# MarineRoboticsGroup/mac

Hardware: AMD Instinct MI355X
Metric: frank_wolfe_iters_per_sec (higher is better)
Workload: dtype f64; 1 GPU; configs[3]: ER N=100000 ~2M candidates, chain fixed, K=10%; N=100000, m_candidates=2001737, K=200173, fixed_edges=99999, fw_iters=209, parallelism=single GPU

## Files before the change

mac_amd/csrc/kernels.h:

```cpp
#pragma once
#include "common.h"

namespace machip {

template <typename T>
struct CsrViewT {
    int n;
    const int* rowptr;
    const int* col;
    const T* val;
};
using CsrView = CsrViewT<double>;

struct PatternView {
    int n;
    const int* prow;
    const int* pcol;
    const int* pk;
    const double* pw;
};

struct LanState {
    int jA;
    int jB;
// ... 17 lines not shown
};

constexpr int kAsmGrid = 4096;
__global__ __launch_bounds__(kBlock) void k_x_bits(const double* __restrict__ x, long m, double tol, unsigned long long* __restrict__ bits) {
    for (long i = (long)blockIdx.x * kBlock + threadIdx.x; i < m; i += (long)gridDim.x * kBlock) {
        const unsigned long long bal = __ballot(x[i] > tol);
        if ((threadIdx.x & 63) == 0) bits[i >> 6] = bal;
    }
}
__device__ __forceinline__ bool x_bit(const unsigned int* __restrict__ bits32, int k) { return (bits32[k >> 5] >> (k & 31)) & 1u; }

template <int G>
__global__ __launch_bounds__(kBlock) void k_asm_count(PatternView P, const unsigned int* __restrict__ xbits,
                                                      int rows_per_block,
                                                      int* __restrict__ cnt, int* __restrict__ blk_sum,
                                                      int* __restrict__ hsum = nullptr) {
    __shared__ int sm[4];
    constexpr int GPB = kBlock / G;
    const int lane = threadIdx.x % G, g = threadIdx.x / G;
    const int r0 = blockIdx.x * rows_per_block;
    const int r1 = min(P.n, r0 + rows_per_block);
    int local = 0, supp = 0, mx = 0;
    for (int r = r0 + g; r < r1; r += GPB) {
        const int b = P.prow[r], e = P.prow[r + 1];
        int c = 0, sc = 0;
        for (int p = b + lane; p < e; p += G) {
            const int k = P.pk[p];
            const bool cand = k >= 0;
            const bool act = cand ? x_bit(xbits, k) : true;
            c += act;
            sc += (cand && act);
        }
// ... 296 lines not shown
    double mx;
    __device__ __forceinline__ void begin(double*) { mx = 0.0; }
    __device__ __forceinline__ double gather(const double* __restrict__ x, int c) const { return x[c]; }
    __device__ __forceinline__ void row(int r, double acc) {
        const double d = dg[r];
        double v = d > 0.0 ? uin[r] + (1.0 - acc) / d : 0.0;
        v = v > 0.0 && v < 1e300 ? v : 0.0;
        uout[r] = v;
        mx = fmax(mx, v);
    }
    __device__ __forceinline__ void end(double* sm) {
        const double m = block_max(mx, sm);
        if (threadIdx.x == 0) pmax[blockIdx.x] = m;
    }
};
__global__ __launch_bounds__(kBlock) void k_land_weight(const double* __restrict__ u, const double* __restrict__ pmax, int npart,
                                                        double* __restrict__ z, int n, double p, double floor_w) {
    __shared__ double sm[4];
    double m = 0.0;
    for (int i = threadIdx.x; i < npart; i += kBlock) m = fmax(m, pmax[i]);
    m = block_max(m, sm);
    if (!(m > 0.0)) return;
    const double inv = 1.0 / m;
    for (int r = blockIdx.x * kBlock + threadIdx.x; r < n; r += gridDim.x * kBlock) {
        const double q = u[r] * inv;
        z[r] *= fmax(q > 0.0 ? exp(p * log(q)) : 0.0, floor_w);
    }
}

__global__ __launch_bounds__(kBlock) void k_lan_update(LanView L) {
    __shared__ double sm[4];
    const int j = L.st->jB;
    const double alpha = reduce_partials(L.part_a, L.P_a, sm);
    const double beta = L.beta[j];
    const double* vj = L.V + (size_t)j * (size_t)L.n;
    const double* vp = j > 0 ? vj - L.n : nullptr;
    double s1 = 0.0, s2 = 0.0, s3 = 0.0;
    for (int r = blockIdx.x * kBlock + threadIdx.x; r < L.n; r += gridDim.x * kBlock) {
        double t = L.w[r] - alpha * vj[r];
        if (vp) t -= beta * vp[r];
        L.u[r] = t;
// ... 658 lines not shown
            else { if (run) atomicAdd(&lh[cur], run); cur = bin; run = 1; }
        }
    }
    if (HIST) {
        if (run) atomicAdd(&lh[cur], run);
        __syncthreads();
        unsigned int* hr = hist0 + (size_t)(blockIdx.x % kSelRep) * kBins;
        for (int i = threadIdx.x; i < kBins; i += kBlock)
            if (lh[i]) atomicAdd(&hr[i], lh[i]);
    }
    if (all.n) peer_drain();
}

template <int BLOCK, class LoadBin>
__device__ __forceinline__ void sel_close_pass(LoadBin load_bin, int pass, unsigned long long prefix, SelState* st,
                                               unsigned int* s_w ) {
    const int tid = threadIdx.x, wv = tid >> 6, ln = tid & 63;
    const int sh = sel_shift(pass), nb = sel_bits(pass);
    const long long kk = pass ? st->kk : st->k;
    const int nbins = 1 << nb;
    constexpr int per = kBins / BLOCK;
    unsigned int c[per];
    unsigned int tsum = 0;
#pragma unroll
    for (int q = 0; q < per; ++q) {
        const int bin = nbins - 1 - (tid * per + q);
        c[q] = bin >= 0 ? load_bin(bin) : 0u;
        tsum += c[q];
    }
    unsigned int x = tsum;
    for (int o = 1; o < 64; o <<= 1) { const unsigned int y = __shfl_up(x, o, kWave); if (ln >= o) x += y; }
    __syncthreads();
    if (ln == 63) s_w[wv] = x;
    __syncthreads();
    for (int q = 0; q < wv; ++q) x += s_w[q];
    const long long pre = (long long)x;
    if (pre >= kk && pre - (long long)tsum < kk) {
        long long rem = kk - (pre - (long long)tsum);
        int q = 0;
        for (; q < per; ++q) {
            if ((long long)c[q] >= rem) break;
            rem -= c[q];
        }
        const int bin = nbins - 1 - (tid * per + q);
        st->kk = rem;
        st->prefix = (prefix << nb) | (unsigned long long)bin;
        if (pass == 5) {
            st->T = (prefix << nb) | (unsigned long long)bin;
            st->cnt_eq = (long long)c[q];
        } else if ((long long)c[q] == rem) {
            st->T = ((prefix << nb) | (unsigned long long)bin) << sh;
            st->cnt_eq = rem;
            st->ticket[7] = 1u;
        }
    }
}

__global__ __launch_bounds__(1024) void k_sel_close0(unsigned int* __restrict__ hist, SelState* st) {
    __shared__ unsigned int s_w[1024 / 64];
    if (st->k <= 0) return;
    const unsigned int* rep = hist + 6 * kBins;
    sel_close_pass<1024>([rep](int bin) {
        unsigned int v[kSelRep];
#pragma unroll
        for (int r = 0; r < kSelRep; ++r) v[r] = rep[(size_t)r * kBins + bin];
        unsigned int a = 0;
#pragma unroll
        for (int r = 0; r < kSelRep; ++r) a += v[r];
        return a; }, 0, 0ull, st, s_w);
}

template <int U, int BLOCK>
__global__ __launch_bounds__(BLOCK) void k_sel_pass(const double* __restrict__ g, long m, int pass,
                                                    unsigned int* __restrict__ hist ,
                                                    SelState* st) {
    __shared__ unsigned int lh[kBins];
    __shared__ unsigned int s_last;
    __shared__ unsigned int s_w[BLOCK / 64];
    const int tid = threadIdx.x;
    if (pass && st->ticket[7]) return;
    for (int i = tid; i < kBins; i += BLOCK) lh[i] = 0;
    __syncthreads();
    const int sh = sel_shift(pass), nb = sel_bits(pass);
    const unsigned long long prefix = pass ? st->prefix : 0ull;
    const unsigned int mask = (1u << nb) - 1u;
    unsigned int cur = 0xffffffffu, run = 0;
    for (long i0 = (long)blockIdx.x * (BLOCK * U) + tid; i0 < m; i0 += (long)gridDim.x * (BLOCK * U)) {
        double gv[U];
#pragma unroll
        for (int q = 0; q < U; ++q) { const long i = i0 + (long)q * BLOCK; gv[q] = g[i < m ? i : m - 1]; }
#pragma unroll
        for (int q = 0; q < U; ++q) {
            if (i0 + (long)q * BLOCK >= m) continue;
            const unsigned long long key = f64_key(gv[q]);
            const bool match = pass == 0 || (key >> (sh + nb)) == prefix;
            if (match) {
                const unsigned int bin = (unsigned int)(key >> sh) & mask;
                if (bin == cur) ++run;
                else {
                    if (run) atomicAdd(&lh[cur], run);
                    cur = bin; run = 1;
                }
            }
        }
    }
    if (run) atomicAdd(&lh[cur], run);
    __syncthreads();
    unsigned int* gh = hist + pass * kBins;
    unsigned int seen = 0;
    for (int i = tid; i < kBins; i += BLOCK)
        if (lh[i]) seen |= __hip_atomic_fetch_add(&gh[i], lh[i], __ATOMIC_RELAXED, __HIP_MEMORY_SCOPE_AGENT);
    asm volatile("" ::"v"(seen));
    __syncthreads();
    if (tid == 0)
        s_last = (__hip_atomic_fetch_add(&st->ticket[pass], 1u, __ATOMIC_ACQ_REL, __HIP_MEMORY_SCOPE_AGENT) == gridDim.x - 1);
    __syncthreads();
    if (!s_last) return;
    sel_close_pass<BLOCK>([gh](int bin) { return __hip_atomic_load(&gh[bin], __ATOMIC_RELAXED, __HIP_MEMORY_SCOPE_AGENT); }, pass, prefix, st, s_w);
}

__global__ __launch_bounds__(1024) void k_sel_ties(const double* __restrict__ g, long m, SelState* st, int prefer_high) {
    __shared__ int s_cnt[16];
    __shared__ long long s_found;
    const long long need = st->kk;
    const long long eq = st->cnt_eq;
    if (st->k <= 0) { if (threadIdx.x == 0) st->tie_limit = prefer_high ? 0x7fffffffffffffffll : -1; return; }
    if (need >= eq) { if (threadIdx.x == 0) st->tie_limit = prefer_high ? -1 : 0x7fffffffffffffffll; return; }
    const unsigned long long T = st->T;
    const int tid = threadIdx.x, wv = tid >> 6, ln = tid & 63;
    if (tid == 0) s_found = -1;
    long long run = 0;
    for (long base = 0; base < m; base += 1024) {
        const long ii = base + tid;
        const long i = prefer_high ? m - 1 - ii : ii;
        const bool is = ii < m && f64_key(g[i]) == T;
        const unsigned long long bal = __ballot(is);
        __syncthreads();
        if (ln == 0) s_cnt[wv] = __popcll(bal);
        __syncthreads();
        int before = 0, tot = 0;
        for (int q = 0; q < 16; ++q) { if (q < wv) before += s_cnt[q]; tot += s_cnt[q]; }
        if (run + tot >= need) {
            const int rank = before + __popcll(bal & ((1ull << ln) - 1ull));
            if (is && run + rank + 1 == need) s_found = i;
            __syncthreads();
            if (tid == 0) st->tie_limit = s_found;
            return;
        }
        run += tot;
    }
    if (tid == 0) st->tie_limit = prefer_high ? -1 : 0x7fffffffffffffffll;
}

constexpr long kSelSmallMax = 32768;
__global__ __launch_bounds__(1024) void k_sel_small(const double* __restrict__ g, long m, long long k, SelState* st, int prefer_high) {
    __shared__ unsigned int lh[kBins];
    __shared__ unsigned int s_w[16];
    __shared__ unsigned long long s_prefix, s_T;
    __shared__ long long s_kk, s_eq, s_found;
    __shared__ int s_done, s_cnt[16];
    const int tid = threadIdx.x, wv = tid >> 6, ln = tid & 63;
    if (tid == 0) { s_prefix = 0; s_T = 0; s_kk = k; s_eq = 0; s_done = 0; s_found = -1; }
    __syncthreads();
    for (int pass = 0; pass < 6 && k > 0; ++pass) {
        if (s_done) break;
        for (int i = tid; i < kBins; i += 1024) lh[i] = 0;
// ... 55 lines not shown
        int before = 0, tot = 0;
        for (int q = 0; q < 16; ++q) { if (q < wv) before += s_cnt[q]; tot += s_cnt[q]; }
        if (runs + tot >= need) {
            const int rank = before + __popcll(bal & ((1ull << ln) - 1ull));
            if (is && runs + rank + 1 == need) s_found = i;
            __syncthreads();
            if (tid == 0) st->tie_limit = s_found;
            return;
        }
        runs += tot;
    }
    if (tid == 0) st->tie_limit = prefer_high ? -1 : 0x7fffffffffffffffll;
}

__global__ __launch_bounds__(kBlock) void k_fw_final(const double* __restrict__ g, const double* __restrict__ x,
                                                     long m, const SelState* __restrict__ st, double gamma,
                                                     double* __restrict__ x_next, double* __restrict__ s_out,
                                                     double* __restrict__ part ,
                                                     double tol = 0.0, unsigned long long* __restrict__ xbits_next = nullptr) {
#pragma clang fp contract(off)
    __shared__ double sm[4];
    const unsigned long long T = st->T;
    const long long lim = st->tie_limit;
    const bool none = st->k <= 0;
    double d = 0.0, q = 0.0;
    for (long i = (long)blockIdx.x * kBlock + threadIdx.x; i < m; i += (long)gridDim.x * kBlock) {
        const double gi = g[i];
        const unsigned long long key = f64_key(gi);
        const double s = (!none && (key > T || (key == T && (long long)i <= lim))) ? 1.0 : 0.0;
        if (s_out) s_out[i] = s;
        if (x) {
            const double xi = x[i];
            const double diff = s - xi;
            d += gi * diff;
            q += gi * gi;
            if (x_next) {
                const double step = gamma * diff;
                const double xn = xi + step;
                x_next[i] = xn;
// ... 80 lines not shown
```

mac_amd/csrc/machip.hip:

```cpp
#include <rccl/rccl.h>
#include <unistd.h>

#include <algorithm>
#include <atomic>
#include <cmath>
#include <chrono>
#include <condition_variable>
#include <functional>
#include <future>
#include <memory>
#include <mutex>
#include <numeric>
#include <thread>
#include <vector>

#include "solver.h"
#include "esp.h"
#include "eig.h"

namespace machip {
thread_local std::string g_err;
}
using namespace machip;

// ... 62 lines not shown
    int *ci = nullptr, *cj = nullptr;
    double* cw = nullptr;
    double *x = nullptr, *x_next = nullptr, *g = nullptr, *s = nullptr, *scratch_m = nullptr;
    int *cnt = nullptr, *blk_sum = nullptr, *rowptr = nullptr, *col = nullptr;
    double *val = nullptr, *blk_lnorm = nullptr;
    unsigned long long *xb = nullptr, *xb_next = nullptr;
    bool xb_valid = false, xb_next_valid = false;
    long nnz = 0, support = 0;
    int maxlen = 0;
    double lnorm = 0.0;
    bool assembled = false, have_vec = false, csr_only = false;
    bool band_dups_ok = true;
    unsigned int* hist = nullptr;
    SelState* sel = nullptr;
    double* part_fw = nullptr;
    int* h_int = nullptr;
    double* h_dbl = nullptr;
    int* d_hint = nullptr;
    double* d_hdbl = nullptr;
    Solver sol;
    ncclComm_t comm = nullptr;
    std::shared_ptr<LocalGroup> lgroup;
    bool first_collective_pending = false;
    hipEvent_t ev_g0 = nullptr, ev_g1 = nullptr, ev_g2 = nullptr;
    bool ev_g_valid = false;
    std::unique_ptr<IpcGroup> ipcg;
    int rank = 0, nranks = 1;
    bool is_lane = false, lane_fw_ready = false;
    std::vector<machip_problem*> lanes;
    unsigned long start_version = 0;
// ... 105 lines not shown
    if (nblk < 1) nblk = 1;
    long rpb = ((long)n + nblk - 1) / nblk;
    rpb = (rpb + gpb - 1) / gpb * gpb;
    p->asm_rpb = (int)rpb;
    p->asm_grid = (int)(((long)n + rpb - 1) / rpb);
    if (p->asm_grid < 1) p->asm_grid = 1;
    if ((rpb + 1) * (long)sizeof(int) > 64 * 1024)
        return fail(MACHIP_BAD_ARG, "num_nodes above the supported 16.7 million (row-offset scan of the assembly kernel)");
    return MACHIP_OK;
}

template <int G>
void launch_asm(machip_problem* p, const PanSpec& S) {
    const PatternView P = p->pattern();
    const unsigned int* xb32 = reinterpret_cast<const unsigned int*>(p->xb);
    k_asm_count<G><<<p->asm_grid, kBlock, 0, p->stream>>>(P, xb32, p->asm_rpb, p->cnt, p->blk_sum, p->d_hint);
    const size_t lds = sizeof(int) * ((size_t)p->asm_rpb + 1);
    k_asm_fill<G><<<p->asm_grid, kBlock, lds, p->stream>>>(P, xb32, p->x, p->asm_rpb, p->cnt, p->blk_sum,
                                                           p->rowptr, p->col, p->val, p->d_hdbl, S);
}

int assemble(machip_problem* p) {
    if (p->csr_only) return fail(MACHIP_BAD_ARG, "handle wraps a caller CSR; nothing to assemble");
    PanSpec S;
    ST_TRY(p->sol.pan_spec_prepare(&S));
    if (!p->xb_valid) {
        const int grid = std::max(1, (int)std::min<long>(kMaxGrid, (p->m + kBlock - 1) / kBlock));
        k_x_bits<<<grid, kBlock, 0, p->stream>>>(p->x, p->m, p->tol_sel, p->xb);
        p->xb_valid = true;
    }
    switch (p->asm_G) {
// ... 15 lines not shown
    }
    p->nnz = nnz; p->support = supp / 2; p->lnorm = ln; p->maxlen = maxlen;
    p->assembled = true;
    return MACHIP_OK;
}

int alloc_common(machip_problem* p, int vbudget_mb = 0) {
    ST_TRY(p->sol.init(p->n, p->stream, vbudget_mb));
    HIP_TRY(hipHostMalloc((void**)&p->h_int, sizeof(int) * 3 * kAsmGrid, hipHostMallocMapped));
    HIP_TRY(hipHostMalloc((void**)&p->h_dbl, sizeof(double) * std::max(4 * kMaxGrid, kAsmGrid), hipHostMallocMapped));
    HIP_TRY(hipHostGetDevicePointer((void**)&p->d_hint, p->h_int, 0));
    HIP_TRY(hipHostGetDevicePointer((void**)&p->d_hdbl, p->h_dbl, 0));
    return MACHIP_OK;
}

int select_on(machip_problem* p, const double* keys, long k, SelState* st, int prefer_high, bool hist0_done = false) {
    const Options& opt = p->sol.opt;
    const long m = p->m;
    if (k < 0) k = 0;
    if (k > m) k = m;
    if (m <= kSelSmallMax && OPT(sel_small, 1)) {
        k_sel_small<<<1, 1024, 0, p->stream>>>(keys, m, (long long)k, st, prefer_high);
        HIP_TRY(hipGetLastError());
        return MACHIP_OK;
    }
    if (!hist0_done) k_sel_init<<<1, 1024, 0, p->stream>>>(st, (long long)k, p->hist, 6 * kBins);
    if (k > 0) {
        constexpr int B = 1024, U = 4;
        const int grid = (int)std::max<long>(1, std::min<long>(128, (m + (long)B * U - 1) / ((long)B * U)));
        if (hist0_done) k_sel_close0<<<1, 1024, 0, p->stream>>>(p->hist, st);
        for (int pass = hist0_done ? 1 : 0; pass < 6; ++pass) k_sel_pass<U, B><<<grid, B, 0, p->stream>>>(keys, m, pass, p->hist, st);
    }
    k_sel_ties<<<1, 1024, 0, p->stream>>>(keys, m, st, prefer_high);
    HIP_TRY(hipGetLastError());
    return MACHIP_OK;
}

int select_topk(machip_problem* p, long k, bool hist0_done = false) { return select_on(p, p->g, k, p->sel, 0, hist0_done); }

void shard_plan(long m, int nranks, int rank, long* lo, long* hi, long* shard) {
    const long sh = nranks > 0 ? (m + nranks - 1) / nranks : m;
    *shard = sh;
    *lo = std::min(m, sh * rank);
    *hi = std::min(m, *lo + sh);
}

int local_allgather(machip_problem* p, long shard) {
    LocalGroup& G = *p->lgroup;
    HIP_TRY(hipStreamSynchronize(p->stream));
    if (!G.barrier()) return fail(MACHIP_RCCL_ERROR, "in-process communicator was shut down by another rank");
    for (int r = 0; r < G.nranks; ++r)
        if (r != p->rank)
            HIP_TRY(hipMemcpyAsync(p->g + shard * r, G.g[(size_t)r] + shard * r, sizeof(double) * (size_t)shard,
// ... 14 lines not shown
        k_ipc_pubwait<<<1, 64, 0, p->stream>>>(p->ipcg->view, 3);
    }
    const bool timed = p->nranks > 1;
    if (timed) {
        if (!p->ev_g0) { HIP_TRY(hipEventCreate(&p->ev_g0)); HIP_TRY(hipEventCreate(&p->ev_g1)); HIP_TRY(hipEventCreate(&p->ev_g2)); }
        p->ev_g_valid = false;
        HIP_TRY(hipEventRecord(p->ev_g0, p->stream));
    }
    if (hi > lo) {
        const int grid = (int)std::min<long>(kMaxGrid * 4, (hi - lo + kBlock - 1) / kBlock);
        PeerVecs all;
        if (ipc_gather) { all.n = p->ipcg->nranks; for (int q = 0; q < all.n; ++q) all.v[q] = p->ipcg->g[q]; }
        const bool fuse = fuse_k > 0 && p->nranks <= 1 && m > kSelSmallMax && OPT(sel_fuse, 1) != 0;
        if (fused) *fused = fuse;
        if (fuse) {
            k_sel_init<<<1, 1024, 0, p->stream>>>(p->sel, (long long)std::min(fuse_k, m), p->hist, (6 + kSelRep) * kBins);
            k_grad<true><<<grid, kBlock, 0, p->stream>>>(p->ci, p->cj, p->cw, p->sol.yvec, lo, hi, p->g, all, p->hist + 6 * kBins);
        } else k_grad<false><<<grid, kBlock, 0, p->stream>>>(p->ci, p->cj, p->cw, p->sol.yvec, lo, hi, p->g, all);
        HIP_TRY(hipGetLastError());
    }
    if (timed) HIP_TRY(hipEventRecord(p->ev_g1, p->stream));
    if (ipc_gather) {
        k_ipc_pubwait<<<1, 64, 0, p->stream>>>(p->ipcg->view, 2);
        HIP_TRY(hipGetLastError());
        HIP_TRY(hipEventRecord(p->ev_g2, p->stream));
        p->ev_g_valid = true;
        return MACHIP_OK;
    }
    if (p->nranks > 1) {
        if (p->comm) {
            NCCL_TRY(ncclAllGather(p->g + shard * p->rank, p->g, (size_t)shard, ncclDouble, p->comm, p->stream));
// ... 286 lines not shown
}

int machip_fw_step(machip_problem* p, int64_t k, int iter, double tol, int max_steps, int warm_start,
                   double* f, double* dual, double* gnorm, machip_solve_stats* stats) {
    if (!p || p->csr_only || !f || !dual || !gnorm) return fail(MACHIP_BAD_ARG, "bad argument");
    GroupGuard guard{p};
    HIP_TRY(hipSetDevice(p->device));
    ST_TRY(assemble(p));
    double lam = 0.0;
    const int grid = std::max(1, (int)std::min<long>(kMaxGrid, (p->m + kBlock - 1) / kBlock));
    const double gamma = 2.0 / ((double)iter + 2.0);
    int epi_status = MACHIP_OK;
    auto epilogue = [&](bool speculative) {
        bool fused = false;
        int st = compute_gradient(p, speculative, (long)k, &fused);
        if (st == MACHIP_OK) st = select_topk(p, (long)k, fused);
        if (st == MACHIP_OK) {
            k_fw_final<<<grid, kBlock, 0, p->stream>>>(p->g, p->x, p->m, p->sel, gamma, p->x_next, nullptr, p->d_hdbl, p->tol_sel, p->xb_next);
            p->xb_next_valid = true;
            if (hipGetLastError() != hipSuccess) st = fail(MACHIP_HIP_ERROR, "k_fw_final launch failed");
        }
        epi_status = st;
    };
    bool done = false;
    auto soft = [](int st) { return st == MACHIP_NOT_CONVERGED || st == MACHIP_DISCONNECTED; };
    if (p->lgroup && p->lgroup->shard_eig) {
        const int st = group_fiedler(p, tol, max_steps, warm_start, &lam, stats);
        if (st != MACHIP_OK) { guard.ok = soft(st); return st; }
    } else {
        const bool spec = p->nranks <= 1 && p->sol.opt.get(kOpt_spec_epilogue, 1) != 0;
        if (spec) p->sol.after_check = [&] { epilogue(true); };
        const int st = run_fiedler(p, tol, max_steps, nullptr, warm_start, &lam, stats);
        p->sol.after_check = nullptr;
        if (st != MACHIP_OK) { guard.ok = soft(st); return st; }
        done = spec && p->sol.hook_seq == p->sol.final_check_seq && epi_status == MACHIP_OK;
// ... 1061 lines not shown
```

mac_amd/csrc/options.h:

```cpp
#pragma once
#include <climits>
#include <cstdlib>
#include <cstring>
#include <mutex>
#include <string>

namespace machip {

#define MACHIP_OPTION_LIST(X)                                                                                                      \
                                                                                                          \
    X(solver) X(graph) X(debug) X(chunk) X(chunk_near) X(sched) X(near_x10) X(trigger_pct) X(classic_n) X(persist) X(pchunk)      \
    X(spec_epilogue) X(spec_slack_pct) X(f32_switch_e9) X(tailless) X(stream) X(stream_trigger_pct) X(stream_retry_pct) X(stream_look) X(stream_margin) X(stream_window) X(stream_far) X(start_land) X(start_pow) X(start_floor_e6) X(start_land_pr_permille) X(start_land_min_mean10)                                                                \
                                                                        \
    X(spmv) X(g) X(unroll) X(block) X(maxgrid) X(defer) X(tpr) X(ell)                                                              \
                                                                                                            \
    X(panel) X(panel_min_n) X(panel_min_mean10) X(panel_multi_min_mean10) X(panel_np) X(panel_nb) X(panel_b2) X(panel_g2)         \
    X(panel_cells) X(panel_maxcells) X(panel_band) X(panel_u) X(panel_u_amp) X(pan32) X(pan32_switch_e9) X(panel_ops) X(panel_rev)                                                                               \
                                                                                                 \
    X(woodbury) X(wb_max) X(wb_hard) X(wb_lane_max) X(exact_big) X(exact_switch) X(gj_look_min) X(lob_density_pct) X(lob_chunk)   \
    X(lob_patience) X(lob_small_s) X(lob_fuse)                                                                                     \
     \
    X(sel_small) X(sel_fuse) X(asm_g) X(asm_maxgrid) X(vbudget_mb) X(vcap) X(lanes) X(lane_vbudget_mb) X(lane_queues) X(shard_eig) X(ipc_panel) \
    X(rccl_timeout_s)

enum OptId {
#define X(n) kOpt_##n,
    MACHIP_OPTION_LIST(X)
#undef X
    kNumOpts
};

constexpr long kOptAuto = LONG_MIN;

inline const char* const* option_names() {
    static const char* const names[] = {
#define X(n) #n,
        MACHIP_OPTION_LIST(X)
#undef X
// ... 53 lines not shown
```

mac_amd/csrc/panel_u.h:

```cpp
#pragma once
#include "panel.h"
#ifndef PAN_U_AHEAD
#define PAN_U_AHEAD 2
#endif

namespace machip {

typedef double pan_f2 __attribute__((ext_vector_type(2)));

struct PanU {
    double* U0;
    double* U1;
    double* W;
    double* sig;
};

__host__ __device__ constexpr int pan_u_rows(int TW) { return 64 * kPanWork * TW; }
__host__ __device__ constexpr int pan_u_cols(int LPT, int TW) {
    return ((2 * kPanWorkThreads * LPT) < ((163840 - 8 * pan_u_rows(TW) - 256) / 8) ? (2 * kPanWorkThreads * LPT) : ((163840 - 8 * pan_u_rows(TW) - 256) / 8)) & ~1;
}

#define PAN_MUL8_ARGS(P, U, L, jrel) (((jrel) & 1) ? (U).U1 : (U).U0), (P).tptr, (P).thead, (P).bval, (P).bcol, (P).n, (P).C, ((P).NP | ((P).TWW << 16)), (((P).NTB << 16) | ((P).rev << 15)), (P), (L), (jrel)
#define PAN_MUL8_ARGS_AT(P, U, L, jrel, b_first) (((jrel) & 1) ? (U).U1 : (U).U0), (P).tptr, (P).thead, (P).bval, (P).bcol, (P).n, (P).C, ((P).NP | ((P).TWW << 16)), ((b_first) | ((P).NTB << 16) | ((P).rev << 15)), (P), (L), (jrel)

// ... 278 lines not shown
        s1 += t; s2 += t * t;
    }
    s1 = block_sum(s1, sm); s2 = block_sum(s2, sm);
    if (threadIdx.x == 0) {
        for (int q = 0; q < kNP; ++q) L.part[q * kMaxGrid + blockIdx.x] = 0.0;
        L.part[0 * kMaxGrid + blockIdx.x] = s2;
        L.part[3 * kMaxGrid + blockIdx.x] = s1;
        if (blockIdx.x == 0) {
            L.st->jA = 0; L.st->jN = 0; L.st->epoch = epoch;
            U.sig[0] = 0.0; U.sig[1] = 0.0;
            U.U0[L.n] = 0.0; U.U0[L.n + 1] = 0.0; U.U1[L.n] = 0.0; U.U1[L.n + 1] = 0.0;
        }
    }
}

}
```

mac_amd/csrc/solver.h:

```cpp
#pragma once
#include <functional>
#include <dlfcn.h>

#include <array>
#include <deque>
#include <limits>
#include <map>
#include <mutex>
#include <tuple>
#include <vector>

#include "kernels.h"
#include "persist.h"
#include "precond.h"
#include "woodbury.h"
#include "panel.h"
#include "plan.h"
#include "tridiag.h"
#include "follow.h"

namespace machip {


struct IpcGroup {
// ... 213 lines not shown
    template <class Op>
    void panel_spmv(const double* x, const Op& op, int grid) {
        const int g1 = pan.NB * pan.NP;
        const PipeView L = pview(SpmvPlan());
        switch (pan.LPT * 10 + pan.TWT) {
#define MACHIP_PANU_CASE(LP, TW) case LP * 10 + TW: k_pan_mul8<LP, TW, double><<<g1, kPanThreads, 0, stream>>>(x, panv.tptr, panv.thead, panv.bval, panv.bcol, panv.n, panv.C, panv.NP | (panv.TWW << 16), panv.NTB << 16, panv, L, -1); break;
#define MACHIP_PANU_ROW(LP) MACHIP_PANU_CASE(LP, 3) MACHIP_PANU_CASE(LP, 5) MACHIP_PANU_CASE(LP, 8)
            MACHIP_PANU_ROW(1) MACHIP_PANU_ROW(2) MACHIP_PANU_ROW(3) MACHIP_PANU_ROW(4) MACHIP_PANU_ROW(5) MACHIP_PANU_ROW(6)
            MACHIP_PANU_ROW(7) MACHIP_PANU_ROW(8) MACHIP_PANU_CASE(9, 3)
#undef MACHIP_PANU_ROW
#undef MACHIP_PANU_CASE
            default: break;
        }
        k_pan_rowop<Op><<<grid, kBlock, 0, stream>>>(panv, x, op);
    }
    int landscape_start(const CsrView& A, const SpmvPlan& pl) {
        const int sweeps = std::min(16, OPT(start_land, 3));
        if (sweeps <= 0) return MACHIP_OK;
        const double pw = (double)std::max(1, OPT(start_pow, 128));
        int gmax = pl.grid;
        const double* f = landscape_field(A, pl, sweeps, &gmax);
        const double floor_w = 1e-6 * (double)std::max(0, OPT(start_floor_e6, 1000));
        k_land_weight<<<vgrid(), kBlock, 0, stream>>>(f, part_c, gmax, u, n, pw, floor_w);
        HIP_TRY(hipGetLastError());
        return MACHIP_OK;
    }
    int vgrid() const { return (int)std::min<long>(kMaxGrid, ((long)n + kBlock - 1) / kBlock); }

    template <typename T = double>
    PipeViewT<T> pview(const SpmvPlan& pl) const {
        PipeViewT<T> L;
        L.n = n; L.st = st; L.Z0 = reinterpret_cast<ZRec<T>*>(Z0); L.Z1 = reinterpret_cast<ZRec<T>*>(Z1); L.V = reinterpret_cast<T*>(V); L.tri = tri; L.htri = d_htri; L.hflag = d_hflag; L.part = part; L.P = pl.grid; L.chunk = 0; L.pub = 0; L.pubstep = 0;
        L.sig = (pl.variant == kPanel && pan_u) ? pu_sig : nullptr;
        return L;
    }
    LanView check_view(const SpmvPlan& pl) const {
        LanView L;
        L.n = n; L.st = st2; L.u = y_raw; L.w = w2; L.V = yvec; L.alpha = scratch3; L.beta = scratch3 + 2;
// ... 44 lines not shown
            case 5: k_lan_persist<5, T><<<1, kPersistThreads, 0, stream>>>(ppack, L, steps); break;
            default: k_lan_persist<6, T><<<1, kPersistThreads, 0, stream>>>(ppack, L, steps); break;
        }
    }
    void launch_persist(const CsrView& A, int steps, bool f32 = false) {
        if (f32) launch_persist_t<float>(A, steps); else launch_persist_t<double>(A, steps);
    }

    int pan_spec_prepare(PanSpec* out) {
        *out = PanSpec();
        pan_rows_ready = false;
        if (!pan_allowed || !pat.prow) return MACHIP_OK;
        const PanPlan sh = plan_panel(opt, n, 0, 1, true, (long)csr_cap, true, OPT(stream, 1) != 0);
        if (!sh.on) return MACHIP_OK;
        ST_TRY(pan_row_buffers(sh, sh.band));
        HIP_TRY(hipMemsetAsync(panv.ovf, 0, sizeof(int), stream));
        out->NP = sh.NP; out->C = sh.C; out->band = sh.band ? 1 : 0;
        out->ps = panv.ps; out->bd = panv.bd; out->bpk = panv.bpk; out->ovf = panv.ovf;
        pan_rows_ready = true; pan_rows_NP = sh.NP; pan_rows_C = sh.C; pan_rows_band = sh.band;
        return MACHIP_OK;
    }
    template <class T>
    int pan_regrow(T** ptr, size_t count, bool* dropped) {
        if (*ptr) { if (!*dropped) { HIP_TRY(hipStreamSynchronize(stream)); drop_graphs(); *dropped = true; } (void)hipFree(*ptr); *ptr = nullptr; }
        return dev_alloc(ptr, count);
    }
    int pan_row_buffers(const PanPlan& pn, bool band) {
        bool dropped = false;
        if ((size_t)pn.NP * (size_t)n > pan_y_cap) {
            ST_TRY(pan_regrow(&panv.ypart, (size_t)pn.NP * ((size_t)n + 2), &dropped));
            ST_TRY(pan_regrow(&panv.ps, ((size_t)pn.NP + 1) * (size_t)n, &dropped));
// ... 853 lines not shown
        int status = MACHIP_NOT_CONVERGED;
        bool switch_out = false;
        double lam = 0.0, res = 0.0;
        const double tiny_l = (lnorm > 0 ? lnorm : 1.0);
        if (n < 2) { *lambda2 = 0.0; return fail(MACHIP_BAD_ARG, "graph with a single node has no Fiedler pair"); }

        const bool pmode_early = OPT(persist, 1) != 0 && chain_like && persist_fits(n, nnz - n - 2 * chain_edges);
        const double* begin_src = nullptr;
        const bool land_local = last_pr <= 0.0 || last_pr <= 0.001 * (double)std::max(1, OPT(start_land_pr_permille, 20)) * (double)n;
        const bool land_dense = 10.0 * (double)nnz >= (double)std::max(0, OPT(start_land_min_mean10, 60)) * (double)n;
        const bool land_ok = !start_guess && !pmode_early && n > OPT(classic_n, 256) && OPT(start_land, 3) > 0 && land_local && land_dense;
        bool warm = start_mode == 1 && have_prev;
        if (warm && land_ok && warm_skip > 0) { --warm_skip; warm = false; }
        const bool warm_probe = warm && land_ok;
        double start_overlap = -1.0;
        if (warm) {
            if (pmode_early) begin_src = yvec;
            else HIP_TRY(hipMemcpyAsync(u, yvec, sizeof(double) * (size_t)n, hipMemcpyDeviceToDevice, stream));
        } else if (have_start) {
            if (pmode_early) begin_src = start;
            else HIP_TRY(hipMemcpyAsync(u, start, sizeof(double) * (size_t)n, hipMemcpyDeviceToDevice, stream));
        } else {
            k_fill_start<<<g2, kBlock, 0, stream>>>(u, n, 0x1234567ull);
        }

        pan_live = false;

        const int chunk0 = std::min(kMaxChunk, std::max(2, OPT(chunk, 32) & ~1));
        const int chunk_near = std::min(chunk0, std::max(2, OPT(chunk_near, 8) & ~1));
        if (max_steps & 1) ++max_steps;
        const double trigger_slack = 0.01 * OPT(trigger_pct, 110);
        const double near_factor = 0.1 * OPT(near_x10, 20);
        std::deque<Pending> pend;
        bool done = false;

// ... 37 lines not shown
                pan_u = true;
                if (precision == 1 && !use_graph(launch_us_hist[kPanel] > 0.0 ? launch_us_hist[kPanel] : 8.0)) {
                    if (pan_bv32_cap < pan_cap) {
                        HIP_TRY(hipStreamSynchronize(stream));
                        if (pan_bv32) (void)hipFree(pan_bv32);
                        pan_bv32 = nullptr; pan_bv32_cap = 0;
                        ST_TRY(dev_alloc(&pan_bv32, pan_cap));
                        pan_bv32_cap = pan_cap;
                    }
                    k_to_f32<<<(int)std::min<long>(kMaxGrid, ((long)pan_cap + kBlock - 1) / kBlock), kBlock, 0, stream>>>(panv.bval, pan_bv32, (long)pan_cap);
                    pan32 = true;
                }
            }
        }
        pan_live = pan.on && pan_u;
        if (!warm && land_ok) ST_TRY(landscape_start(A, landscape_plan(nnz)));
        {
            const int vk = std::max(0, std::min(7, (int)pp.variant));
            cur_launch_us = launch_us_hist[vk] > 0.0 ? launch_us_hist[vk] : (pp.variant == kPanel ? 8.0 : 4.2 + 2e-6 * (double)nnz);
        }
        if (OPT(debug, 0)) fprintf(stderr, "[machip] fused steps: variant %d, %.2f us per launch (%s) -> %s\n", (int)pp.variant, cur_launch_us, launch_us_hist[std::max(0, std::min(7, (int)pp.variant))] > 0.0 ? "measured" : "model", use_graph(cur_launch_us) ? "captured chunks" : "eager launches");
        const PipeView L = pview(pp);
        const int pchunk0 = std::min(kPersistMaxSteps, std::max(2, OPT(pchunk, 64)));
        const bool debug = OPT(debug, 0) != 0;
        bool f32_seq = precision == 1 && !classic && pp.variant == kVec;
        const double f32_switch = std::max(std::max(tol, 1e-9 * (double)OPT(f32_switch_e9, 2000)),
                                           3e-7 * std::sqrt((double)n));
        long steps_lowp = 0;
        if (f32_seq && !pmode) {
            if (valf_cap < (size_t)nnz) {
                HIP_TRY(hipStreamSynchronize(stream));
// ... 10 lines not shown
        if (pmode) ST_TRY(pack_persist(A));
        while (!done && steps_total < max_steps) {
            seq_sharded = false; seq_ipc = false;
            pan32_from = INT_MAX;
            if (pmode) {
                ++epoch;
                k_persist_begin<<<g2, kBlock, 0, stream>>>(persist_view(), (int)epoch, begin_src);
                begin_src = nullptr;
            } else if (classic) {
                k_vec_sums<<<g2, kBlock, 0, stream>>>(u, n, part_u);
                k_set_state<<<1, 64, 0, stream>>>(stc, 0);
            } else if (f32_seq) {
                ++epoch;
                k_pipe_init<<<pp.grid, kBlock, 0, stream>>>(pview<float>(pp), u, (int)epoch);
            } else {
                ++epoch;
                if (pan_u) k_pipe_init_u<<<pp.grid, kBlock, 0, stream>>>(L, pu, u, (int)epoch);
                else k_pipe_init<<<pp.grid, kBlock, 0, stream>>>(L, u, (int)epoch);
                if (shard && pp.variant == kVec) {
                    seq_sharded = true; seq_plan = pp;
                    ST_TRY(shard_broadcast_init());
                } else if (ipc && precision == 0 && ((pp.variant == kVec && pp.grid >= ipc->nranks) || (pp.variant == kPanel && pan_u))) {
                    seq_sharded = true; seq_ipc = true; seq_plan = pp;
                }
            }
            const double seq_tol = f32_seq ? f32_switch : tol;
            int J_enq = 0;
            int prev_tailless = 0;
            const bool tail_ok = !pmode && !classic && !seq_sharded && OPT(tailless, 1) != 0;
            int J_timed = 0;
            HIP_TRY(hipEventRecord(evs0, stream));
            ha.clear(); hb.assign(1, 0.0); hl1.assign(1, 0.0);
            guess.clear();
// ... 463 lines not shown
```

Baseline: 132.4 iter/s.

## Fold auxiliary clears, selection init and tie scan into neighboring kernels

Adds a fold_aux option, on by default, that removes several small launches per Frank-Wolfe iteration and eigen-start. The histogram and ticket clears move into k_fw_final, and the overflow memset moves into k_asm_count. Selection state init is folded into k_sel_close0, and the tie scan runs in the last block of the final select pass. The landscape weighting now reads the start vector directly, skipping a device copy, and fuses the pipeline init into one kernel. The cost is extra branching, state carried across calls through a sel_clean flag, and a single-block tie scan inside the pass kernel.

```diff
diff --git a/mac_amd/csrc/kernels.h b/mac_amd/csrc/kernels.h
--- a/mac_amd/csrc/kernels.h
+++ b/mac_amd/csrc/kernels.h
@@ -55,8 +55,9 @@
 __global__ __launch_bounds__(kBlock) void k_asm_count(PatternView P, const unsigned int* __restrict__ xbits,
                                                       int rows_per_block,
                                                       int* __restrict__ cnt, int* __restrict__ blk_sum,
-                                                      int* __restrict__ hsum = nullptr) {
+                                                      int* __restrict__ hsum = nullptr, int* __restrict__ ovf_clear = nullptr) {
     __shared__ int sm[4];
+    if (ovf_clear && blockIdx.x == 0 && threadIdx.x == 0) *ovf_clear = 0;
     constexpr int GPB = kBlock / G;
     const int lane = threadIdx.x % G, g = threadIdx.x / G;
     const int r0 = blockIdx.x * rows_per_block;
@@ -383,17 +384,21 @@
         if (threadIdx.x == 0) pmax[blockIdx.x] = m;
     }
 };
+__device__ __forceinline__ double land_weight(double ur, double m, double p, double floor_w) {
+    const double inv = 1.0 / m;
+    const double q = ur * inv;
+    return fmax(q > 0.0 ? exp(p * log(q)) : 0.0, floor_w);
+}
 __global__ __launch_bounds__(kBlock) void k_land_weight(const double* __restrict__ u, const double* __restrict__ pmax, int npart,
-                                                        double* __restrict__ z, int n, double p, double floor_w) {
+                                                        const double* src, double* z, int n, double p, double floor_w) {
     __shared__ double sm[4];
     double m = 0.0;
     for (int i = threadIdx.x; i < npart; i += kBlock) m = fmax(m, pmax[i]);
     m = block_max(m, sm);
-    if (!(m > 0.0)) return;
-    const double inv = 1.0 / m;
+    if (!(m > 0.0) && src == z) return;
     for (int r = blockIdx.x * kBlock + threadIdx.x; r < n; r += gridDim.x * kBlock) {
-        const double q = u[r] * inv;
-        z[r] *= fmax(q > 0.0 ? exp(p * log(q)) : 0.0, floor_w);
+#pragma clang fp contract(off)
+        z[r] = m > 0.0 ? src[r] * land_weight(u[r], m, p, floor_w) : src[r];
     }
 }
 
@@ -1082,10 +1087,10 @@
 
 template <int BLOCK, class LoadBin>
 __device__ __forceinline__ void sel_close_pass(LoadBin load_bin, int pass, unsigned long long prefix, SelState* st,
-                                               unsigned int* s_w ) {
+                                               unsigned int* s_w , long long kk,
+                                               int tie_mode = -1, long long* s_scan = nullptr) {
     const int tid = threadIdx.x, wv = tid >> 6, ln = tid & 63;
     const int sh = sel_shift(pass), nb = sel_bits(pass);
-    const long long kk = pass ? st->kk : st->k;
     const int nbins = 1 << nb;
     constexpr int per = kBins / BLOCK;
     unsigned int c[per];
@@ -1113,20 +1118,30 @@
         const int bin = nbins - 1 - (tid * per + q);
         st->kk = rem;
         st->prefix = (prefix << nb) | (unsigned long long)bin;
+        const long long all_ties = tie_mode == 1 ? -1 : 0x7fffffffffffffffll;
         if (pass == 5) {
             st->T = (prefix << nb) | (unsigned long long)bin;
             st->cnt_eq = (long long)c[q];
+            if (tie_mode >= 0) {
+                if (rem >= (long long)c[q]) st->tie_limit = all_ties;
+                else { s_scan[0] = 1; s_scan[1] = rem; s_scan[2] = (long long)((prefix << nb) | (unsigned long long)bin); }
+            }
         } else if ((long long)c[q] == rem) {
             st->T = ((prefix << nb) | (unsigned long long)bin) << sh;
             st->cnt_eq = rem;
             st->ticket[7] = 1u;
-        }
-    }
-}
-
-__global__ __launch_bounds__(1024) void k_sel_close0(unsigned int* __restrict__ hist, SelState* st) {
+            if (tie_mode >= 0) st->tie_limit = all_ties;
+        }
+    }
+}
+
+__global__ __launch_bounds__(1024) void k_sel_close0(unsigned int* __restrict__ hist, SelState* st, long long k_init = -1, int tie_mode = -1) {
     __shared__ unsigned int s_w[1024 / 64];
-    if (st->k <= 0) return;
+    if (k_init >= 0) {
+        if (threadIdx.x == 0) { st->prefix = 0; st->kk = k_init; st->cnt_eq = 0; st->T = 0; st->tie_limit = -1; st->k = k_init; }
+        if (k_init == 0) return;
+    } else if (st->k <= 0) return;
+    const long long kk = k_init >= 0 ? k_init : st->k;
     const unsigned int* rep = hist + 6 * kBins;
     sel_close_pass<1024>([rep](int bin) {
         unsigned int v[kSelRep];
@@ -1135,68 +1150,13 @@
         unsigned int a = 0;
 #pragma unroll
         for (int r = 0; r < kSelRep; ++r) a += v[r];
-        return a; }, 0, 0ull, st, s_w);
-}
-
-template <int U, int BLOCK>
-__global__ __launch_bounds__(BLOCK) void k_sel_pass(const double* __restrict__ g, long m, int pass,
-                                                    unsigned int* __restrict__ hist ,
-                                                    SelState* st) {
-    __shared__ unsigned int lh[kBins];
-    __shared__ unsigned int s_last;
-    __shared__ unsigned int s_w[BLOCK / 64];
-    const int tid = threadIdx.x;
-    if (pass && st->ticket[7]) return;
-    for (int i = tid; i < kBins; i += BLOCK) lh[i] = 0;
-    __syncthreads();
-    const int sh = sel_shift(pass), nb = sel_bits(pass);
-    const unsigned long long prefix = pass ? st->prefix : 0ull;
-    const unsigned int mask = (1u << nb) - 1u;
-    unsigned int cur = 0xffffffffu, run = 0;
-    for (long i0 = (long)blockIdx.x * (BLOCK * U) + tid; i0 < m; i0 += (long)gridDim.x * (BLOCK * U)) {
-        double gv[U];
-#pragma unroll
-        for (int q = 0; q < U; ++q) { const long i = i0 + (long)q * BLOCK; gv[q] = g[i < m ? i : m - 1]; }
-#pragma unroll
-        for (int q = 0; q < U; ++q) {
-            if (i0 + (long)q * BLOCK >= m) continue;
-            const unsigned long long key = f64_key(gv[q]);
-            const bool match = pass == 0 || (key >> (sh + nb)) == prefix;
-            if (match) {
-                const unsigned int bin = (unsigned int)(key >> sh) & mask;
-                if (bin == cur) ++run;
-                else {
-                    if (run) atomicAdd(&lh[cur], run);
-                    cur = bin; run = 1;
-                }
-            }
-        }
-    }
-    if (run) atomicAdd(&lh[cur], run);
-    __syncthreads();
-    unsigned int* gh = hist + pass * kBins;
-    unsigned int seen = 0;
-    for (int i = tid; i < kBins; i += BLOCK)
-        if (lh[i]) seen |= __hip_atomic_fetch_add(&gh[i], lh[i], __ATOMIC_RELAXED, __HIP_MEMORY_SCOPE_AGENT);
-    asm volatile("" ::"v"(seen));
-    __syncthreads();
-    if (tid == 0)
-        s_last = (__hip_atomic_fetch_add(&st->ticket[pass], 1u, __ATOMIC_ACQ_REL, __HIP_MEMORY_SCOPE_AGENT) == gridDim.x - 1);
-    __syncthreads();
-    if (!s_last) return;
-    sel_close_pass<BLOCK>([gh](int bin) { return __hip_atomic_load(&gh[bin], __ATOMIC_RELAXED, __HIP_MEMORY_SCOPE_AGENT); }, pass, prefix, st, s_w);
-}
-
-__global__ __launch_bounds__(1024) void k_sel_ties(const double* __restrict__ g, long m, SelState* st, int prefer_high) {
-    __shared__ int s_cnt[16];
-    __shared__ long long s_found;
-    const long long need = st->kk;
-    const long long eq = st->cnt_eq;
-    if (st->k <= 0) { if (threadIdx.x == 0) st->tie_limit = prefer_high ? 0x7fffffffffffffffll : -1; return; }
-    if (need >= eq) { if (threadIdx.x == 0) st->tie_limit = prefer_high ? -1 : 0x7fffffffffffffffll; return; }
-    const unsigned long long T = st->T;
+        return a; }, 0, 0ull, st, s_w, kk, tie_mode);
+}
+
+__device__ __forceinline__ void sel_tie_scan(const double* __restrict__ g, long m, SelState* st, int prefer_high, long long need,
+                                             unsigned long long T, int* s_cnt , long long* s_found) {
     const int tid = threadIdx.x, wv = tid >> 6, ln = tid & 63;
-    if (tid == 0) s_found = -1;
+    if (tid == 0) *s_found = -1;
     long long run = 0;
     for (long base = 0; base < m; base += 1024) {
         const long ii = base + tid;
@@ -1210,14 +1170,81 @@
         for (int q = 0; q < 16; ++q) { if (q < wv) before += s_cnt[q]; tot += s_cnt[q]; }
         if (run + tot >= need) {
             const int rank = before + __popcll(bal & ((1ull << ln) - 1ull));
-            if (is && run + rank + 1 == need) s_found = i;
+            if (is && run + rank + 1 == need) *s_found = i;
             __syncthreads();
-            if (tid == 0) st->tie_limit = s_found;
+            if (tid == 0) st->tie_limit = *s_found;
             return;
         }
         run += tot;
     }
     if (tid == 0) st->tie_limit = prefer_high ? -1 : 0x7fffffffffffffffll;
+}
+
+template <int U, int BLOCK>
+__global__ __launch_bounds__(BLOCK) void k_sel_pass(const double* __restrict__ g, long m, int pass,
+                                                    unsigned int* __restrict__ hist ,
+                                                    SelState* st, int tie_mode = -1) {
+    static_assert(BLOCK == 1024, "sel_tie_scan walks the keys with 16 waves");
+    __shared__ unsigned int lh[kBins];
+    __shared__ unsigned int s_last;
+    __shared__ unsigned int s_w[BLOCK / 64];
+    __shared__ long long s_scan[3], s_found;
+    __shared__ int s_cnt[16];
+    const int tid = threadIdx.x;
+    if (pass && st->ticket[7]) return;
+    for (int i = tid; i < kBins; i += BLOCK) lh[i] = 0;
+    __syncthreads();
+    const int sh = sel_shift(pass), nb = sel_bits(pass);
+    const unsigned long long prefix = pass ? st->prefix : 0ull;
+    const unsigned int mask = (1u << nb) - 1u;
+    unsigned int cur = 0xffffffffu, run = 0;
+    for (long i0 = (long)blockIdx.x * (BLOCK * U) + tid; i0 < m; i0 += (long)gridDim.x * (BLOCK * U)) {
+        double gv[U];
+#pragma unroll
+        for (int q = 0; q < U; ++q) { const long i = i0 + (long)q * BLOCK; gv[q] = g[i < m ? i : m - 1]; }
+#pragma unroll
+        for (int q = 0; q < U; ++q) {
+            if (i0 + (long)q * BLOCK >= m) continue;
+            const unsigned long long key = f64_key(gv[q]);
+            const bool match = pass == 0 || (key >> (sh + nb)) == prefix;
+            if (match) {
+                const unsigned int bin = (unsigned int)(key >> sh) & mask;
+                if (bin == cur) ++run;
+                else {
+                    if (run) atomicAdd(&lh[cur], run);
+                    cur = bin; run = 1;
+                }
+            }
+        }
+    }
+    if (run) atomicAdd(&lh[cur], run);
+    __syncthreads();
+    unsigned int* gh = hist + pass * kBins;
+    unsigned int seen = 0;
+    for (int i = tid; i < kBins; i += BLOCK)
+        if (lh[i]) seen |= __hip_atomic_fetch_add(&gh[i], lh[i], __ATOMIC_RELAXED, __HIP_MEMORY_SCOPE_AGENT);
+    asm volatile("" ::"v"(seen));
+    __syncthreads();
+    if (tid == 0)
+        s_last = (__hip_atomic_fetch_add(&st->ticket[pass], 1u, __ATOMIC_ACQ_REL, __HIP_MEMORY_SCOPE_AGENT) == gridDim.x - 1);
+    __syncthreads();
+    if (!s_last) return;
+    if (tid == 0) s_scan[0] = 0;
+    sel_close_pass<BLOCK>([gh](int bin) { return __hip_atomic_load(&gh[bin], __ATOMIC_RELAXED, __HIP_MEMORY_SCOPE_AGENT); }, pass, prefix, st, s_w,
+                          pass ? st->kk : st->k, tie_mode, s_scan);
+    if (tie_mode < 0) return;
+    __syncthreads();
+    if (s_scan[0]) sel_tie_scan(g, m, st, tie_mode, s_scan[1], (unsigned long long)s_scan[2], s_cnt, &s_found);
+}
+
+__global__ __launch_bounds__(1024) void k_sel_ties(const double* __restrict__ g, long m, SelState* st, int prefer_high) {
+    __shared__ int s_cnt[16];
+    __shared__ long long s_found;
+    const long long need = st->kk;
+    const long long eq = st->cnt_eq;
+    if (st->k <= 0) { if (threadIdx.x == 0) st->tie_limit = prefer_high ? 0x7fffffffffffffffll : -1; return; }
+    if (need >= eq) { if (threadIdx.x == 0) st->tie_limit = prefer_high ? -1 : 0x7fffffffffffffffll; return; }
+    sel_tie_scan(g, m, st, prefer_high, need, st->T, s_cnt, &s_found);
 }
 
 constexpr long kSelSmallMax = 32768;
@@ -1303,15 +1330,19 @@
 }
 
 __global__ __launch_bounds__(kBlock) void k_fw_final(const double* __restrict__ g, const double* __restrict__ x,
-                                                     long m, const SelState* __restrict__ st, double gamma,
+                                                     long m, const SelState* st, double gamma,
                                                      double* __restrict__ x_next, double* __restrict__ s_out,
                                                      double* __restrict__ part ,
-                                                     double tol = 0.0, unsigned long long* __restrict__ xbits_next = nullptr) {
+                                                     double tol = 0.0, unsigned long long* __restrict__ xbits_next = nullptr,
+                                                     unsigned int* __restrict__ hist_clear = nullptr, int nclear = 0,
+                                                     unsigned int* ticket_clear = nullptr) {
 #pragma clang fp contract(off)
     __shared__ double sm[4];
     const unsigned long long T = st->T;
     const long long lim = st->tie_limit;
     const bool none = st->k <= 0;
+    for (int i = blockIdx.x * kBlock + threadIdx.x; i < nclear; i += gridDim.x * kBlock) hist_clear[i] = 0u;
+    if (ticket_clear && blockIdx.x == 0 && threadIdx.x < 8) ticket_clear[threadIdx.x] = 0u;
     double d = 0.0, q = 0.0;
     for (long i = (long)blockIdx.x * kBlock + threadIdx.x; i < m; i += (long)gridDim.x * kBlock) {
         const double gi = g[i];
diff --git a/mac_amd/csrc/machip.hip b/mac_amd/csrc/machip.hip
--- a/mac_amd/csrc/machip.hip
+++ b/mac_amd/csrc/machip.hip
@@ -100,6 +100,7 @@
     unsigned int* hist = nullptr;
     SelState* sel = nullptr;
     double* part_fw = nullptr;
+    bool sel_clean = false;
     int* h_int = nullptr;
     double* h_dbl = nullptr;
     int* d_hint = nullptr;
@@ -235,7 +236,8 @@
 void launch_asm(machip_problem* p, const PanSpec& S) {
     const PatternView P = p->pattern();
     const unsigned int* xb32 = reinterpret_cast<const unsigned int*>(p->xb);
-    k_asm_count<G><<<p->asm_grid, kBlock, 0, p->stream>>>(P, xb32, p->asm_rpb, p->cnt, p->blk_sum, p->d_hint);
+    int* ovf_clear = (S.NP && p->sol.opt.get(kOpt_fold_aux, 1) != 0) ? S.ovf : nullptr;
+    k_asm_count<G><<<p->asm_grid, kBlock, 0, p->stream>>>(P, xb32, p->asm_rpb, p->cnt, p->blk_sum, p->d_hint, ovf_clear);
     const size_t lds = sizeof(int) * ((size_t)p->asm_rpb + 1);
     k_asm_fill<G><<<p->asm_grid, kBlock, lds, p->stream>>>(P, xb32, p->x, p->asm_rpb, p->cnt, p->blk_sum,
                                                            p->rowptr, p->col, p->val, p->d_hdbl, S);
@@ -281,11 +283,20 @@
     return MACHIP_OK;
 }
 
-int select_on(machip_problem* p, const double* keys, long k, SelState* st, int prefer_high, bool hist0_done = false) {
+int select_on(machip_problem* p, const double* keys, long k, SelState* st, int prefer_high, bool hist0_done = false, bool folded = false) {
     const Options& opt = p->sol.opt;
     const long m = p->m;
     if (k < 0) k = 0;
     if (k > m) k = m;
+    p->sel_clean = false;
+    if (hist0_done && folded) {
+        constexpr int B = 1024, U = 4;
+        const int grid = (int)std::max<long>(1, std::min<long>(128, (m + (long)B * U - 1) / ((long)B * U)));
+        k_sel_close0<<<1, 1024, 0, p->stream>>>(p->hist, st, (long long)k, prefer_high);
+        if (k > 0) for (int pass = 1; pass < 6; ++pass) k_sel_pass<U, B><<<grid, B, 0, p->stream>>>(keys, m, pass, p->hist, st, prefer_high);
+        HIP_TRY(hipGetLastError());
+        return MACHIP_OK;
+    }
     if (m <= kSelSmallMax && OPT(sel_small, 1)) {
         k_sel_small<<<1, 1024, 0, p->stream>>>(keys, m, (long long)k, st, prefer_high);
         HIP_TRY(hipGetLastError());
@@ -303,7 +314,7 @@
     return MACHIP_OK;
 }
 
-int select_topk(machip_problem* p, long k, bool hist0_done = false) { return select_on(p, p->g, k, p->sel, 0, hist0_done); }
+int select_topk(machip_problem* p, long k, bool hist0_done = false, bool folded = false) { return select_on(p, p->g, k, p->sel, 0, hist0_done, folded); }
 
 void shard_plan(long m, int nranks, int rank, long* lo, long* hi, long* shard) {
     const long sh = nranks > 0 ? (m + nranks - 1) / nranks : m;
@@ -348,7 +359,9 @@
         const bool fuse = fuse_k > 0 && p->nranks <= 1 && m > kSelSmallMax && OPT(sel_fuse, 1) != 0;
         if (fused) *fused = fuse;
         if (fuse) {
-            k_sel_init<<<1, 1024, 0, p->stream>>>(p->sel, (long long)std::min(fuse_k, m), p->hist, (6 + kSelRep) * kBins);
+            if (!(OPT(fold_aux, 1) != 0 && p->sel_clean))
+                k_sel_init<<<1, 1024, 0, p->stream>>>(p->sel, (long long)std::min(fuse_k, m), p->hist, (6 + kSelRep) * kBins);
+            p->sel_clean = false;
             k_grad<true><<<grid, kBlock, 0, p->stream>>>(p->ci, p->cj, p->cw, p->sol.yvec, lo, hi, p->g, all, p->hist + 6 * kBins);
         } else k_grad<false><<<grid, kBlock, 0, p->stream>>>(p->ci, p->cj, p->cw, p->sol.yvec, lo, hi, p->g, all);
         HIP_TRY(hipGetLastError());
@@ -665,11 +678,15 @@
     auto epilogue = [&](bool speculative) {
         bool fused = false;
         int st = compute_gradient(p, speculative, (long)k, &fused);
-        if (st == MACHIP_OK) st = select_topk(p, (long)k, fused);
+        const bool folded = fused && p->sol.opt.get(kOpt_fold_aux, 1) != 0;
+        if (st == MACHIP_OK) st = select_topk(p, (long)k, fused, folded);
         if (st == MACHIP_OK) {
-            k_fw_final<<<grid, kBlock, 0, p->stream>>>(p->g, p->x, p->m, p->sel, gamma, p->x_next, nullptr, p->d_hdbl, p->tol_sel, p->xb_next);
+            if (folded) k_fw_final<<<grid, kBlock, 0, p->stream>>>(p->g, p->x, p->m, p->sel, gamma, p->x_next, nullptr, p->d_hdbl, p->tol_sel, p->xb_next,
+                                                                   p->hist, (6 + kSelRep) * kBins, p->sel->ticket);
+            else k_fw_final<<<grid, kBlock, 0, p->stream>>>(p->g, p->x, p->m, p->sel, gamma, p->x_next, nullptr, p->d_hdbl, p->tol_sel, p->xb_next);
             p->xb_next_valid = true;
             if (hipGetLastError() != hipSuccess) st = fail(MACHIP_HIP_ERROR, "k_fw_final launch failed");
+            else if (folded) p->sel_clean = true;
         }
         epi_status = st;
     };
diff --git a/mac_amd/csrc/options.h b/mac_amd/csrc/options.h
--- a/mac_amd/csrc/options.h
+++ b/mac_amd/csrc/options.h
@@ -21,7 +21,9 @@
     X(lob_patience) X(lob_small_s) X(lob_fuse)                                                                                     \
      \
     X(sel_small) X(sel_fuse) X(asm_g) X(asm_maxgrid) X(vbudget_mb) X(vcap) X(lanes) X(lane_vbudget_mb) X(lane_queues) X(shard_eig) X(ipc_panel) \
-    X(rccl_timeout_s)
+    X(rccl_timeout_s)                                                                                                              \
+              \
+    X(fold_aux)
 
 enum OptId {
 #define X(n) kOpt_##n,
diff --git a/mac_amd/csrc/panel_u.h b/mac_amd/csrc/panel_u.h
--- a/mac_amd/csrc/panel_u.h
+++ b/mac_amd/csrc/panel_u.h
@@ -316,4 +316,35 @@
     }
 }
 
-}
+__global__ __launch_bounds__(kBlock) void k_land_weight_init_u(const double* __restrict__ f, const double* __restrict__ pmax, int npart,
+                                                               const double* src, double* z, double p, double floor_w,
+                                                               PipeView L, PanU U, int epoch) {
+    __shared__ double sm[4];
+    double m = 0.0;
+    for (int i = threadIdx.x; i < npart; i += kBlock) m = fmax(m, pmax[i]);
+    m = block_max(m, sm);
+    double s1 = 0.0, s2 = 0.0;
+    for (int r = blockIdx.x * kBlock + threadIdx.x; r < L.n; r += gridDim.x * kBlock) {
+        double t;
+        {
+#pragma clang fp contract(off)
+            t = m > 0.0 ? src[r] * land_weight(f[r], m, p, floor_w) : src[r];
+        }
+        z[r] = t;
+        U.U0[r] = t;
+        s1 += t; s2 += t * t;
+    }
+    s1 = block_sum(s1, sm); s2 = block_sum(s2, sm);
+    if (threadIdx.x == 0) {
+        for (int q = 0; q < kNP; ++q) L.part[q * kMaxGrid + blockIdx.x] = 0.0;
+        L.part[0 * kMaxGrid + blockIdx.x] = s2;
+        L.part[3 * kMaxGrid + blockIdx.x] = s1;
+        if (blockIdx.x == 0) {
+            L.st->jA = 0; L.st->jN = 0; L.st->epoch = epoch;
+            U.sig[0] = 0.0; U.sig[1] = 0.0;
+            U.U0[L.n] = 0.0; U.U0[L.n + 1] = 0.0; U.U1[L.n] = 0.0; U.U1[L.n + 1] = 0.0;
+        }
+    }
+}
+
+}
diff --git a/mac_amd/csrc/solver.h b/mac_amd/csrc/solver.h
--- a/mac_amd/csrc/solver.h
+++ b/mac_amd/csrc/solver.h
@@ -251,14 +251,15 @@
         }
         k_pan_rowop<Op><<<grid, kBlock, 0, stream>>>(panv, x, op);
     }
-    int landscape_start(const CsrView& A, const SpmvPlan& pl) {
+    int landscape_start(const CsrView& A, const SpmvPlan& pl, const double* src, const SpmvPlan* init = nullptr) {
         const int sweeps = std::min(16, OPT(start_land, 3));
         if (sweeps <= 0) return MACHIP_OK;
         const double pw = (double)std::max(1, OPT(start_pow, 128));
         int gmax = pl.grid;
         const double* f = landscape_field(A, pl, sweeps, &gmax);
         const double floor_w = 1e-6 * (double)std::max(0, OPT(start_floor_e6, 1000));
-        k_land_weight<<<vgrid(), kBlock, 0, stream>>>(f, part_c, gmax, u, n, pw, floor_w);
+        if (init) k_land_weight_init_u<<<init->grid, kBlock, 0, stream>>>(f, part_c, gmax, src, u, pw, floor_w, pview(*init), pu, (int)epoch);
+        else k_land_weight<<<vgrid(), kBlock, 0, stream>>>(f, part_c, gmax, src, u, n, pw, floor_w);
         HIP_TRY(hipGetLastError());
         return MACHIP_OK;
     }
@@ -333,7 +334,7 @@
         const PanPlan sh = plan_panel(opt, n, 0, 1, true, (long)csr_cap, true, OPT(stream, 1) != 0);
         if (!sh.on) return MACHIP_OK;
         ST_TRY(pan_row_buffers(sh, sh.band));
-        HIP_TRY(hipMemsetAsync(panv.ovf, 0, sizeof(int), stream));
+        if (OPT(fold_aux, 1) == 0) HIP_TRY(hipMemsetAsync(panv.ovf, 0, sizeof(int), stream));
         out->NP = sh.NP; out->C = sh.C; out->band = sh.band ? 1 : 0;
         out->ps = panv.ps; out->bd = panv.bd; out->bpk = panv.bpk; out->ovf = panv.ovf;
         pan_rows_ready = true; pan_rows_NP = sh.NP; pan_rows_C = sh.C; pan_rows_band = sh.band;
@@ -1217,11 +1218,14 @@
         if (warm && land_ok && warm_skip > 0) { --warm_skip; warm = false; }
         const bool warm_probe = warm && land_ok;
         double start_overlap = -1.0;
+        const bool fold = OPT(fold_aux, 1) != 0;
+        const double* land_src = u;
         if (warm) {
             if (pmode_early) begin_src = yvec;
             else HIP_TRY(hipMemcpyAsync(u, yvec, sizeof(double) * (size_t)n, hipMemcpyDeviceToDevice, stream));
         } else if (have_start) {
             if (pmode_early) begin_src = start;
+            else if (fold && land_ok) land_src = start;
             else HIP_TRY(hipMemcpyAsync(u, start, sizeof(double) * (size_t)n, hipMemcpyDeviceToDevice, stream));
         } else {
             k_fill_start<<<g2, kBlock, 0, stream>>>(u, n, 0x1234567ull);
@@ -1289,7 +1293,13 @@
             }
         }
         pan_live = pan.on && pan_u;
-        if (!warm && land_ok) ST_TRY(landscape_start(A, landscape_plan(nnz)));
+        bool seq_started = false;
+        if (!warm && land_ok) {
+            const bool with_init = fold && pan_u && precision == 0 && !shard && !ipc && !classic;
+            if (with_init) ++epoch;
+            ST_TRY(landscape_start(A, landscape_plan(nnz), land_src, with_init ? &pp : nullptr));
+            seq_started = with_init;
+        }
         {
             const int vk = std::max(0, std::min(7, (int)pp.variant));
             cur_launch_us = launch_us_hist[vk] > 0.0 ? launch_us_hist[vk] : (pp.variant == kPanel ? 8.0 : 4.2 + 2e-6 * (double)nnz);
@@ -1330,9 +1340,12 @@
                 ++epoch;
                 k_pipe_init<<<pp.grid, kBlock, 0, stream>>>(pview<float>(pp), u, (int)epoch);
             } else {
-                ++epoch;
-                if (pan_u) k_pipe_init_u<<<pp.grid, kBlock, 0, stream>>>(L, pu, u, (int)epoch);
-                else k_pipe_init<<<pp.grid, kBlock, 0, stream>>>(L, u, (int)epoch);
+                if (seq_started) seq_started = false;
+                else {
+                    ++epoch;
+                    if (pan_u) k_pipe_init_u<<<pp.grid, kBlock, 0, stream>>>(L, pu, u, (int)epoch);
+                    else k_pipe_init<<<pp.grid, kBlock, 0, stream>>>(L, u, (int)epoch);
+                }
                 if (shard && pp.variant == kVec) {
                     seq_sharded = true; seq_plan = pp;
                     ST_TRY(shard_broadcast_init());
```

After: 134.4 iter/s, median of 2. No clear change (+1.5%).
